# JettHuang/jet-pbrt

Hardware: AMD Instinct MI355X
Metric: Msamples/sec (whole node) + per-pixel L2 vs CPU ref, cornell_box 1024spp (higher is better)
Workload: dtype f32

## Files before the change

jet-pbrt_amd/csrc/jp_kernels.hip:

```cpp
#include "jp_common.h"
#include "jp_tex.h"
#include "jp_normals.h"
#include "jp_normal_map.h"
#include "jp_env.h"
#include "jp_mis.h"
#include "jp_lens.h"
#include "jp_xbsdf.h"
#include "jp_film.h"

#include <cstdio>
#include <cstring>
#include <string>
#include <vector>
#include <algorithm>
#include <cmath>
#include <mutex>
#include <thread>
#include "jp_devmem.h"
#include "jp_lbvh.h"
#include "jp_ploc.h"

struct NoLens {};
template <bool kLens> struct LensArg { typedef NoLens type; };
template <> struct LensArg<true> { typedef JpLensPlan type; };
// ... 155 lines not shown
		const float4 co = ro, cd = rd;
		if (j + JP_BLOCK < n) { ro = q.ray_o[cur][i + JP_BLOCK]; rd = q.ray_d[cur][i + JP_BLOCK]; }
		float tmax = JP_INF;
		int hit;
		if constexpr (kMode == 2) hit = acc.trace_unbounded(sc, xyz(co), xyz(cd), 0.001f, tmax);
		else hit = acc.template trace<false>(sc, xyz(co), xyz(cd), 0.001f, tmax);
		q.hit[i] = make_float2(tmax, __int_as_float(hit));
		h += hit >= 0 ? 1u : 0u;
	}
	for (int off = 32; off > 0; off >>= 1) h += __shfl_down(h, off);
	if ((threadIdx.x & 63) == 0 && h) atomicAdd(&cnt->closest_hit, (unsigned long long)h);
}

#ifndef JP_SHADE_TILE
#define JP_SHADE_TILE 8192
#endif
template <bool kSmooth> struct SmoothVars { };
template <> struct SmoothVars<true> { float4 next, rec; V3 Ns; bool on, guard; };
template <bool kSmooth> __device__ __forceinline__ V3 shade_n(const SmoothVars<kSmooth>& sm, V3 N) { if constexpr (kSmooth) return sm.Ns; else return N; }
template <bool kSmooth> __device__ __forceinline__ bool shade_refuses(const SmoothVars<kSmooth>& sm, V3 w, V3 wo, V3 Ng)
{
	if constexpr (kSmooth) return sm.guard && dot(w, Ng) * dot(wo, Ng) <= 0.f; else return false;
}
template <bool kTab, bool kPrims, bool kStage, bool kSort, bool kTex, bool kPick, bool kEnv, bool kMis, typename F = FeatAll, bool kOne = false, bool kSmooth = false>
__device__ __forceinline__ void shade_body(SceneView sc, Queues q, RenderConst rc, int cur, DevCounters* cnt, const TexView& tv, const PickView& pv, const EnvView& ev, const MisView& mv, const NormView& nv = NormView())
{
	static_assert(kPick || !kMis, "k_shade: the light strategy's pdf needs the light table");
	static_assert(kTab || !kPrims, "k_shade: primitive records in LDS only together with the tables");
	static_assert(kPick || !kEnv, "k_shade: the map light is an entry of the light table");
	static_assert(!kSmooth || !kPrims, "k_shade: a shading normal has no entry in the frame table");
	constexpr int kWaves = JP_BLOCK / 64, kMaxSeg = (JP_SHADE_TILE / JP_BLOCK) * kWaves;
	static_assert(JP_SHADE_TILE % JP_BLOCK == 0 && JP_SHADE_TILE <= 65536, "k_shade: tile positions are 16-bit");
	__shared__ unsigned short s_idx[kSort ? JP_SHADE_TILE : 1];
	static_assert(!kOne || (kSort && kPrims && !F::delta && !F::other_lights && !kTex && !kPick && !kMis), "k_shade: the one-sweep partition is the lean sorted instance's");
	__shared__ unsigned char s_key[kSort && !kOne ? JP_SHADE_TILE : 1];
	__shared__ unsigned int s_cnt[kSort && !kOne ? JP_SHADE_CLASSES * kMaxSeg : 1];
	__shared__ unsigned int s_two;
	__shared__ unsigned int s_wsum[kWaves];
	__shared__ unsigned int s_ctr[3];
	const unsigned int lane = threadIdx.x & 63u;
	const int n_tab_l = kPick ? 0 : 2 * sc.n_lights;
	const int n_tab = n_tab_l + 4 * sc.n_mats + (sc.n_mats + 3) / 4, n_tab_all = n_tab + (kPrims ? 8 * sc.n_prims : 0);
	float4* s_lights = s_dyn;
	float4* s_mats = s_lights + n_tab_l;
	int* s_mtype = (int*)(s_mats + 4 * sc.n_mats);
	float4* s_prims = s_dyn + n_tab;
	int4* s_meta = (int4*)(s_prims + 4 * sc.n_prims);
	const float4* s_frames = s_prims + 5 * sc.n_prims;
	float4* s_stage = s_dyn + n_tab_all + threadIdx.x;
	const unsigned int b = blockIdx.x, n = q.blk_q[cur][b];
	const int nxt = cur ^ 1;
#ifdef JP_SHADE_TIMING
	unsigned long long t_acc[10] = { 0, 0, 0, 0, 0, 0, 0, 0, 0, 0 }, t_last = __builtin_amdgcn_s_memtime();
#endif
	if (kTab)
	{
		for (int i = threadIdx.x; i < n_tab_all; i += 2 * JP_BLOCK)
		{
			const bool two = i + JP_BLOCK < n_tab_all;
			const float4 a = sc.shade_tab[i], c2 = two ? sc.shade_tab[i + JP_BLOCK] : a;
			s_dyn[i] = a; if (two) s_dyn[i + JP_BLOCK] = c2;
		}
	}
	if (n == 0) { if (threadIdx.x == 0) { q.blk_q[nxt][b] = 0; q.blk_sh[b] = 0; } return; }
	if (threadIdx.x == 0) { s_ctr[0] = 0; s_ctr[1] = 0; s_ctr[2] = 0; if (kOne) s_two = 0; }
	__syncthreads();
	const float4* lights = (kTab && !kPick) ? (const float4*)s_lights : sc.lights;
	const float4* mats = kTab ? (const float4*)s_mats : sc.mats;
	const int* mat_type = kTab ? (const int*)s_mtype : sc.mat_type;
	const float4* prims = kPrims ? (const float4*)s_prims : sc.prims;
	const int4* meta_t = kPrims ? (const int4*)s_meta : sc.meta;
	const unsigned int rbase = b * q.R;
	const unsigned int t0 = 0, count = n;
	JP_TS(0);
	if (kOne)
	{
		const unsigned int tid = threadIdx.x, npass = (count + JP_BLOCK - 1) / JP_BLOCK;
		const unsigned long long ltm = (1ull << lane) - 1ull;
		#pragma unroll 1
		for (unsigned int r0 = 0; r0 < npass; r0 += 8)
		{
			int pi[8];
			#pragma unroll
			for (int u = 0; u < 8; u++)
			{
				const unsigned int j = (r0 + u) * JP_BLOCK + tid;
				pi[u] = j < count ? __float_as_int(q.hit[rbase + t0 + j].y) : -2;
			}
			int mt[8]; unsigned long long ma[8], mb[8];
			unsigned int na = 0, nb = 0;
			#pragma unroll
			for (int u = 0; u < 8; u++)
			{
				mt[u] = -1;
				if (pi[u] >= 0) { const int m = meta_t[pi[u]].y; if (m >= 0) mt[u] = mat_type[m]; }
				ma[u] = __ballot(mt[u] == JP_MAT_MATTE); mb[u] = __ballot(mt[u] == JP_MAT_METAL);
				na += (unsigned int)__popcll(ma[u]); nb += (unsigned int)__popcll(mb[u]);
			}
// ... 74 lines not shown
			for (int i = 0; i < 3; i++) { const unsigned int at = 3 * tid + i; if (at < nctr) s_cnt[at] = base; base += v[i]; }
		}
		__syncthreads();
		#pragma unroll 1
		for (unsigned int r = 0; r < npass; r++)
		{
			const unsigned int key = s_key[r * JP_BLOCK + tid];
			unsigned int pre = 0;
			#pragma unroll
			for (int c = 0; c < JP_SHADE_CLASSES; c++)
			{
				if (!((rc.class_mask >> c) & 1)) continue;
				const unsigned long long m = __ballot(key == (unsigned int)c);
				if (key == (unsigned int)c) pre = (unsigned int)__popcll(m & ltm);
			}
			if (key < JP_SHADE_CLASSES) s_idx[s_cnt[key * seg + r * kWaves + wave] + pre] = (unsigned short)(r * JP_BLOCK + tid);
		}
		__syncthreads();
	}
	SmoothVars<kSmooth> sm;
	if constexpr (kSmooth) sm.next = make_float4(0, 0, 0, 0);
	float4 ro_n = make_float4(0, 0, 0, 0), rd_n = ro_n, rb_n = ro_n; float2 h_n = make_float2(0, 0); unsigned int s_n = 0; float2 m_n = make_float2(0, 0);
	JP_TS(1);
	const unsigned int n_front = kOne ? (s_two & 0xffffu) : 0u, n_back = kOne ? (s_two >> 16) : 0u, fence = ((n_front + 63u) >> 6) << 6;
#define JP_CHUNK_HAS(v)  (kOne ? ((v) < fence ? (v) < n_front : (v) - fence < n_back) : (v) < count)
#define JP_CHUNK_SPOT(v) (kOne ? ((v) < fence ? (v) : count - 1u - ((v) - fence)) : (v))
	const unsigned int nch = kOne ? (fence >> 6) + ((n_back + 63u) >> 6) : (count + 63u) >> 6;
	unsigned int tk = wave_take(&s_ctr[0], 1u);
	unsigned int c0 = (nch - 1u - tk) << 6;
	if (tk < nch && JP_CHUNK_HAS(c0 + lane)) { const unsigned int pos = JP_CHUNK_SPOT(c0 + lane), i0 = rbase + t0 + (kSort ? (unsigned int)s_idx[pos] : pos); ro_n = q.ray_o[cur][i0]; rd_n = q.ray_d[cur][i0]; rb_n = q.beta[cur][i0]; h_n = q.hit[i0]; if (kTex) s_n = tv.side[i0]; if (kMis) m_n = mv.side[cur][i0]; if constexpr (kSmooth) sm.next = nv.side[i0]; }
	while (tk < nch)
	{
		const bool valid = JP_CHUNK_HAS(c0 + lane);
#ifdef JP_SHADE_TIMING
		JP_TS(2);
		asm volatile("s_waitcnt vmcnt(0)" ::: "memory");
		JP_TS(3);
#endif
#ifdef JP_SHADE_NO_PREFETCH
		if (valid) { const unsigned int pos = JP_CHUNK_SPOT(c0 + lane), i0 = rbase + t0 + (kSort ? (unsigned int)s_idx[pos] : pos); ro_n = q.ray_o[cur][i0]; rd_n = q.ray_d[cur][i0]; rb_n = q.beta[cur][i0]; h_n = q.hit[i0]; if (kTex) s_n = tv.side[i0]; if (kMis) m_n = mv.side[cur][i0]; if constexpr (kSmooth) sm.next = nv.side[i0]; }
		const float4 ro = ro_n, rd = rd_n, rb = rb_n; const float2 h = h_n; const unsigned int sw = s_n; const float2 ms = m_n;
		if constexpr (kSmooth) sm.rec = sm.next;
		tk = wave_take(&s_ctr[0], 1u); c0 = (nch - 1u - tk) << 6;
#else
		const float4 ro = ro_n, rd = rd_n, rb = rb_n; const float2 h = h_n; const unsigned int sw = s_n; const float2 ms = m_n;
		if constexpr (kSmooth) sm.rec = sm.next;
		tk = wave_take(&s_ctr[0], 1u); c0 = (nch - 1u - tk) << 6;
		if (tk < nch && JP_CHUNK_HAS(c0 + lane))
		{
			const unsigned int pos = JP_CHUNK_SPOT(c0 + lane);
			const unsigned int i1 = rbase + t0 + (kSort ? (unsigned int)s_idx[pos] : pos);
			ro_n = q.ray_o[cur][i1]; rd_n = q.ray_d[cur][i1]; rb_n = q.beta[cur][i1]; h_n = q.hit[i1]; if (kTex) s_n = tv.side[i1]; if (kMis) m_n = mv.side[cur][i1]; if constexpr (kSmooth) sm.next = nv.side[i1];
		}
#endif
		bool shaded = false, wantNee = false, alive = false;
		V3 o = mk(0, 0, 0), d = mk(0, 0, 1), beta = mk(0, 0, 0), p = mk(0, 0, 0), N = mk(0, 0, 1);
		if constexpr (kSmooth) { sm.Ns = N; sm.on = false; sm.guard = false; }
		int slot = 0, bounce = 0; bool spec = false; unsigned int dim = 0; uint32_t key = 0;
		Closure c; c.kind = CL_LAMBERT; Frame fr; fr.s = fr.t = fr.n = mk(0, 0, 1);
		float2 nm = make_float2(0.f, 0.f);
		if (valid)
		{
			o = xyz(ro); d = xyz(rd); beta = xyz(rb);
			slot = __float_as_int(ro.w); key = (uint32_t)__float_as_int(rb.w);
			const int flags = __float_as_int(rd.w);
			bounce = FLAG_BOUNCE(flags); spec = FLAG_SPEC(flags); dim = FLAG_DIM(flags);
			const int pi = __float_as_int(h.y);
			const bool found = pi >= 0;
			int mat = -1, hitprim = 0; bool nflip = false, tabframe = kPrims;
			V3 Le = splat(0);
			float wLe = 1.f;
			if (found)
			{
				const float4 g3 = prims[4 * pi + 3];
				const int4 meta = meta_t[pi];
				const int type = __float_as_int(g3.w);
				p = o + h.x * d;
				if (type == JP_SHAPE_TRIANGLE) N = xyz(g3);
				else if (!F::curved || type == JP_SHAPE_RECTANGLE) { nflip = !(dot(xyz(g3), d) <= 0); N = nflip ? -xyz(g3) : xyz(g3); }
				else if (type == JP_SHAPE_DISK) N = xyz(prims[4 * pi + 1]);
				else { const float4 g0 = prims[4 * pi]; N = normalize(p - xyz(g0)); tabframe = false; }
				hitprim = pi;
// ... 55 lines not shown
					int l2; V3 Lr;
					if (kEnv) { l2 = ev.light; Lr = xyz(ev.texel[env_lookup(ev, d)]); }
					else { const float4 r4 = pv.env[e]; l2 = __float_as_int(r4.w); Lr = xyz(r4); }
					bool unweighed;
					const float a = light_pdf(sc, prims, lights, pv, ev, kEnv, l2, o, d, 0.f, N, unweighed);
					const float w = a > 0.f ? mis_weight(ms.x, a) : 1.f;
					float4 L = q.lacc[slot];
					V3 s2 = mk(L.x, L.y, L.z) + cmul(beta, Lr) * w;
					q.lacc[slot] = make_float4(s2.x, s2.y, s2.z, 0.f);
				}
			}
			if (!isblack(Le))
			{
				float4 L = q.lacc[slot];
				V3 a = mk(L.x, L.y, L.z) + (kMis ? cmul(beta, Le) * wLe : cmul(beta, Le));
				q.lacc[slot] = make_float4(a.x, a.y, a.z, 0.f);
			}
			if (found && bounce < rc.max_depth)
			{
				if (mat < 0) { alive = true; if (kMis) nm = make_float2(ms.x, ms.y + h.x); }
				else
				{
					float up = 0.f;
					const int mtype = mat_type[mat];
					if constexpr (kSmooth) { sm.on = sm.rec.w != 0.f; sm.Ns = sm.on ? xyz(sm.rec) : N; sm.guard = sm.on && mtype != JP_MAT_GLASS; }
					if (F::delta && mtype == JP_MAT_PLASTIC) up = rngf(rc, key, dim++);
					if (kTex && sw != 0u) make_closure_tex(mats, mtype, mat, up, tex_color(tv, sw), c);
					else make_closure<F>(mats, mtype, mat, up, c);
#ifdef JP_DBG_SKIP_FRAME
					fr.n = N; fr.s = mk(N.y, N.z, N.x); fr.t = mk(N.z, N.x, N.y);
#else
					if (kPrims && (!F::curved || tabframe))
					{
						const float4 fn = s_frames[3 * hitprim], fs = s_frames[3 * hitprim + 1], ft = s_frames[3 * hitprim + 2];
						fr.n = nflip ? -xyz(fn) : xyz(fn); fr.s = xyz(fs); fr.t = nflip ? -xyz(ft) : xyz(ft);
					}
					else fr = frame_from_z(shade_n<kSmooth>(sm, N));
#endif
					shaded = true;
					wantNee = !is_delta<F>(c);
#ifdef JP_DBG_SKIP_NEE
					wantNee = false;
#endif
				}
			}
		}
		JP_TS(4);
// ... 118 lines not shown
				for (int kk = 0; kk < k; kk++)
				{
					q.sh_d[(size_t)kk * q.cap + qs] = s_stage[(2 * kk) * JP_BLOCK];
					q.sh_c[(size_t)kk * q.cap + qs] = s_stage[(2 * kk + 1) * JP_BLOCK];
				}
			}
		}
		else if (ma) j = rbase + wave_take(&s_ctr[1], (unsigned int)__popcll(ma)) + (unsigned int)__popcll(ma & lt);
		if (alive)
		{
			q.ray_o[nxt][j] = make_float4(p.x, p.y, p.z, __int_as_float(slot));
			q.ray_d[nxt][j] = make_float4(nd.x, nd.y, nd.z, __int_as_float(MK_FLAGS(nbounce, nspec, dim)));
			q.beta[nxt][j] = make_float4(nbeta.x, nbeta.y, nbeta.z, __int_as_float((int)key));
			if (kMis) mv.side[nxt][j] = nm;
		}
		JP_TS(7);
#ifdef JP_SHADE_TIMING
		asm volatile("s_waitcnt vmcnt(0)" ::: "memory");
		JP_TS(9);
#endif
	}
#undef JP_CHUNK_HAS
#undef JP_CHUNK_SPOT
	JP_TS(2);
	__syncthreads();
	JP_TS(8);
#ifdef JP_SHADE_TIMING
	if (lane == 0) for (int i = 0; i < 10; i++) atomicAdd(&g_shade_t[i], t_acc[i]);
	if (lane == 0) atomicAdd(&g_shade_t[15], 1ull);
#endif
	if (threadIdx.x == 0)
	{
		const unsigned int run_q = kStage ? (s_ctr[1] & 0xffffu) : s_ctr[1], run_sh = kStage ? (s_ctr[1] >> 16) : s_ctr[2];
		q.blk_q[nxt][b] = run_q; q.blk_sh[b] = run_sh;
		if (run_q) atomicAdd(&cnt->n_queue[nxt], run_q);
		if (run_sh) atomicAdd(&cnt->n_shadow, run_sh);
	}
}
template <bool kTab, bool kPrims, bool kStage, bool kSort, typename F = FeatAll>
__global__ void __launch_bounds__(JP_BLOCK) k_shade(SceneView sc, Queues q, RenderConst rc, int cur, DevCounters* cnt)
{
	const TexView tv = {}; const PickView pv = {}; const EnvView ev = {}; const MisView mv = {};
	shade_body<kTab, kPrims, kStage, kSort, false, false, false, false, F>(sc, q, rc, cur, cnt, tv, pv, ev, mv);
}
__global__ void __launch_bounds__(JP_BLOCK) k_shade_lean_one(SceneView sc, Queues q, RenderConst rc, int cur, DevCounters* cnt)
{
	const TexView tv = {}; const PickView pv = {}; const EnvView ev = {}; const MisView mv = {};
	shade_body<true, true, true, true, false, false, false, false, FeatLean, true>(sc, q, rc, cur, cnt, tv, pv, ev, mv);
}

template <int kMode, typename F = FeatAll>
__global__ void __launch_bounds__(JP_BLOCK, 4) k_shadow(SceneView sc, Queues q, RenderConst rc, int depth, DevCounters* cnt)
{
#ifdef JP_TRAV_TIMING
	unsigned long long t_acc[10] = { 0, 0, 0, 0, 0, 0, 0, 0, 0, 0 }, t_last = __builtin_amdgcn_s_memtime();
#endif
	SceneAccess<kMode, F> acc(sc, depth);
	const unsigned int b = blockIdx.x, E = q.blk_sh[b], rbase = b * q.R;
	JP_TT(0);
	unsigned int rays = 0, occ = 0;
	float4 so_n = make_float4(0, 0, 0, 0), sd_n = make_float4(0, 0, 1, 0);
	if (threadIdx.x < E) { so_n = q.sh_o[rbase + threadIdx.x]; sd_n = q.sh_d[rbase + threadIdx.x]; }
	for (unsigned int j = threadIdx.x; j < E; j += JP_BLOCK)
	{
		const unsigned int e = rbase + j;
#ifdef JP_TRAV_TIMING
		JP_TT(1);
		asm volatile("s_waitcnt vmcnt(0)" ::: "memory");
		JP_TT(2);
#endif
		const float4 so = so_n; float4 sd = sd_n;
// ... 583 lines not shown
```

jet-pbrt_amd/csrc/jp_render.h:

```cpp
#pragma once
namespace
{
enum { CLS_EXTEND = 0, CLS_SHADE = 1, CLS_SHADOW = 2, CLS_OTHER = 3, CLS_PATH = 4, CLS_NORMAL = 5, CLS_NMAP = 6, CLS_TEXEL = 7 };

int lens_plan_of(const JpContext* c, JpLensPlan& lp)
{
	std::memset(&lp, 0, sizeof(lp));
	if (!c->lens_on) return JP_OK;
	if (jp_lens_make_plan(&c->plan.sv.cam, &c->lens, &lp) != 0) return fail(JP_ERR_INVALID_ARGUMENT, "jp_set_lens: the uploaded camera's right / up vectors have no finite positive length");
	return JP_OK;
}

void free_queues(JpContext* c) { c->qb = QueueBufs(); c->cap = 0; c->planes_alloc = 0; c->blk_alloc = 0; }

int ensure_queues(JpContext* c, unsigned int cap, int planes, unsigned int nblocks)
{
	if (c->cap >= cap && c->planes_alloc >= planes && c->blk_alloc >= nblocks) return JP_OK;
	cap = std::max(cap, c->cap); planes = std::max(planes, c->planes_alloc); nblocks = std::max(nblocks, c->blk_alloc);
	free_queues(c);
	auto alloc = [](DevBuf& b, auto*& p, size_t bytes) { return reserve(b, p, bytes) == hipSuccess; };
	Queues& q = c->q; QueueBufs& qb = c->qb; bool ok = true;
	for (int b = 0; b < 2 && ok; b++) ok = alloc(qb.ray_o[b], q.ray_o[b], (size_t)cap * 16) && alloc(qb.ray_d[b], q.ray_d[b], (size_t)cap * 16) && alloc(qb.beta[b], q.beta[b], (size_t)cap * 16)
	                                       && alloc(qb.blk_q[b], q.blk_q[b], (size_t)nblocks * 4);
	ok = ok && alloc(qb.hit, q.hit, (size_t)cap * 8) && alloc(qb.lacc, q.lacc, (size_t)cap * 16) && alloc(qb.sh_o, q.sh_o, (size_t)cap * 16)
// ... 98 lines not shown
}

typedef void (*ShadowKernel)(SceneView, Queues, RenderConst, int, DevCounters*);
typedef void (*ShadowRefillKernel)(SceneView, Queues, RenderConst, int, int*, DevCounters*);
struct ShadowLaunch { ShadowRefillKernel refill; ShadowKernel plain; size_t lds; int words; bool cert_fell_back; };
template <int M> ShadowRefillKernel shadow_refill(const ScenePlan& p)
{
	static const ShadowRefillKernel k[3][2] = { { k_shadow_persist<M, 8, false>, k_shadow_persist<M, 8, true> }, { k_shadow_persist<M, 16, false>, k_shadow_persist<M, 16, true> }, { k_shadow_persist<M, 32, false>, k_shadow_persist<M, 32, true> } };
	return k[refill_row(p)][p.vote];
}
ShadowLaunch shadow_kernel(const ScenePlan& p, unsigned int R, bool generic)
{
	const int words = std::min(shadow_depth(p), p.stack_lds_words);
	const size_t plds = (size_t)words * JP_BLOCK * sizeof(int) + (((size_t)R * p.n_planes + 31) / 32) * 4 * (p.cert ? 2 : 1);
	if (lean_traversal(p, generic)) return { nullptr, k_shadow<2, FeatFlat>, p.lds_bytes, p.stack_depth, p.cert };
	if (!refill_walks(p) || plds > 64 * 1024)
		return { nullptr, p.trav_mode == 3 ? k_shadow<3> : (p.trav_mode == 5 ? k_shadow<5> : (p.trav_mode == 2 ? k_shadow<2> : (p.trav_mode == 1 ? k_shadow<1> : k_shadow<0>))), p.trav_mode == 3 ? p.lds_bytes_shadow : p.lds_bytes, p.stack_depth, p.cert };
	const ShadowRefillKernel k = p.trav_mode == 5 ? (p.cert ? shadow_refill<6>(p) : shadow_refill<5>(p)) : (p.q4_shadow ? shadow_refill<4>(p) : (p.trav_mode == 3 ? shadow_refill<3>(p) : shadow_refill<0>(p)));
	return { k, nullptr, plds, words, false };
}

typedef void (*ShadeKernel)(SceneView, Queues, RenderConst, int, DevCounters*);
typedef void (*ShadeTexKernel)(SceneView, Queues, RenderConst, int, DevCounters*, TexView);
struct ShadeKernels { ShadeKernel plain; ShadeTexKernel tex; };
template <bool kTab, bool kPrims, bool kStage> ShadeKernels shade_row(bool sort)
{
	ShadeKernels k = { sort ? k_shade<kTab, kPrims, kStage, true> : k_shade<kTab, kPrims, kStage, false>, sort ? k_shade_tex<kTab, kPrims, kStage, true> : k_shade_tex<kTab, kPrims, kStage, false> };
	return k;
}
ShadeKernels shade_kernels(const ScenePlan& p, bool generic)
{
	if (lean_shading(p, generic))
	{
		ShadeKernels k = shade_row<true, true, true>(p.shade_sort);
		k.plain = p.shade_sort ? k_shade<true, true, true, true, FeatLean> : k_shade<true, true, true, false, FeatLean>;
#ifndef JP_NO_ONE_SWEEP
		if (p.shade_sort && !p.has_null_material) k.plain = k_shade_lean_one;
#endif
		return k;
	}
	if (p.shade_prims_in_lds) return p.stage_nee ? shade_row<true, true, true>(p.shade_sort) : shade_row<true, true, false>(p.shade_sort);
	if (p.tables_in_lds) return p.stage_nee ? shade_row<true, false, true>(p.shade_sort) : shade_row<true, false, false>(p.shade_sort);
	return shade_row<false, false, false>(p.shade_sort);
}

typedef void (*ShadePickKernel)(SceneView, Queues, RenderConst, int, DevCounters*, PickView);
typedef void (*ShadePickTexKernel)(SceneView, Queues, RenderConst, int, DevCounters*, TexView, PickView);
struct ShadePickKernels { ShadePickKernel plain; ShadePickTexKernel tex; };
ShadePickKernels shade_pick_kernels(const ScenePlan& p);
typedef void (*ShadeEnvKernel)(SceneView, Queues, RenderConst, int, DevCounters*, PickView, EnvView);
typedef void (*ShadeEnvTexKernel)(SceneView, Queues, RenderConst, int, DevCounters*, TexView, PickView, EnvView);
struct ShadeEnvKernels { ShadeEnvKernel plain; ShadeEnvTexKernel tex; };
ShadeEnvKernels shade_env_kernels(const ScenePlan& p);
typedef void (*ShadeMisKernel)(SceneView, Queues, RenderConst, int, DevCounters*, PickView, MisView);
typedef void (*ShadeMisTexKernel)(SceneView, Queues, RenderConst, int, DevCounters*, TexView, PickView, MisView);
typedef void (*ShadeMisEnvKernel)(SceneView, Queues, RenderConst, int, DevCounters*, PickView, EnvView, MisView);
typedef void (*ShadeMisEnvTexKernel)(SceneView, Queues, RenderConst, int, DevCounters*, TexView, PickView, EnvView, MisView);
struct ShadeMisKernels { ShadeMisKernel pick; ShadeMisTexKernel pick_tex; ShadeMisEnvKernel env; ShadeMisEnvTexKernel env_tex; };
ShadeMisKernels shade_mis_kernels(const ScenePlan& p);
struct SmoothKernels
// ... 98 lines not shown
		}
		c->q.cap = cap; c->q.R = R;
		const bool tex = p.textured && rp->integrator == JP_INTEGRATOR_PATH;
		if (tex) if (const int e = reserve_idle(c, c->side, (size_t)cap * sizeof(unsigned int)); e != JP_OK) return e;
		TexView tv = p.tv; tv.side = c->side.get<unsigned int>();
		const bool mis = c->estimator == JP_ESTIMATOR_MIS && rp->integrator == JP_INTEGRATOR_PATH;
		MisView mv = {};
		if (mis) if (const int e = ensure_mis_side(c, cap, mv); e != JP_OK) return e;
		NormView nv = p.nv;
		if (smooth) if (const int e = ensure_normal_side(c, cap, nv); e != JP_OK) return e;
		if (const int e = reserve_idle(c, c->spill, spill_need(p, p.persist ? deepest_walk(p) : 0, G) * sizeof(int)); e != JP_OK) return e;
		if (const int e = reserve_idle(c, c->pix_acc, (size_t)npix * 16); e != JP_OK) return e;
		int* const d_spill = c->spill.get<int>(); float4* const d_pix_acc = c->pix_acc.get<float4>();

		RenderConst rc; rc.width = rp->width; rc.height = rp->height; rc.spp = rp->spp; rc.max_depth = rp->max_depth; rc.seed = rp->seed;
		rc.band_rows = sh.band; rc.shard_index = sh.index; rc.shard_count = sh.count; rc.npix = (int)npix; rc.local_rows = sh.lane_rows; rc.n_planes = p.n_planes;
		rc.lane_index = lane_index; rc.lane_count = lane_count; rc.lane_rows = lane_group; rc.class_mask = p.class_mask; rc.sampler_debug = rp->sampler_mode == JP_SAMPLER_DEBUG ? 1 : 0;
		rc.slot_bits = slot_bits;
		rc.tiled = 0;
		rc.compact = (p.trav_mode != 2 && p.trav_mode != 1 && npix % JP_BLOCK == 0) ? 1 : 0;
		if (c->opt.compact_regions != 0) rc.compact = (c->opt.compact_regions > 0 && npix % JP_BLOCK == 0) ? 1 : 0;
		const int grid = (int)G;
		const bool generic = c->opt.reserved[0] == 1;
		const ExtendLaunch ek = extend_kernel(p, generic); const ShadowLaunch sk = shadow_kernel(p, R, generic); const ShadeKernels hk = shade_kernels(p, generic); const OtherKernel ok = other_kernel(p);
		const ShadePickKernels pk = p.pick ? shade_pick_kernels(p) : ShadePickKernels{ nullptr, nullptr };
		const ShadeEnvKernels vk = p.env ? shade_env_kernels(p) : ShadeEnvKernels{ nullptr, nullptr };
		const ShadeMisKernels mk2 = mis ? shade_mis_kernels(p) : ShadeMisKernels{ nullptr, nullptr, nullptr, nullptr };
		const SmoothKernels nk = smooth ? shade_smooth_kernels(p) : SmoothKernels{};
		JpLensPlan lp;
		if (const int e = lens_plan_of(c, lp); e != JP_OK) return e;
		for (int s0 = 0; s0 < rp->spp; s0 += sbatch)
		{
			rc.s0 = s0; rc.sbatch = std::min(sbatch, rp->spp - s0);
			{
				Stamper t(c, CLS_OTHER);
				if (c->lens_on) hipLaunchKernelGGL(k_raygen<true>, dim3(grid), dim3(JP_BLOCK), 0, c->stream, p.sv, c->q, rc, d_cnt, lp);
				else hipLaunchKernelGGL(k_raygen<false>, dim3(grid), dim3(JP_BLOCK), 0, c->stream, p.sv, c->q, rc, d_cnt, NoLens());
			}
			if (rp->integrator != JP_INTEGRATOR_PATH)
			{
				Stamper t(c, CLS_OTHER);
				const int ogrid = (int)std::min<unsigned int>((P + JP_BLOCK - 1) / JP_BLOCK, (unsigned int)(c->n_cus * 16));
				hipLaunchKernelGGL(ok, dim3(ogrid), dim3(JP_BLOCK), p.lds_bytes, c->stream, p.sv, c->q, rc, rp->integrator, p.stack_depth, d_cnt, c->lens_on ? 1 : 0, lp);
			}
			int cur = 0;
			int iters = rp->integrator != JP_INTEGRATOR_PATH ? 0 : rp->max_depth + 1;
			for (int it = 0;; it++)
			{
				if (it >= iters)
				{
					if (rp->integrator != JP_INTEGRATOR_PATH || !p.has_null_material || it > iters + 64) break;
// ... 21 lines not shown
							else if (p.env) hipLaunchKernelGGL(nk.env_tex, dim3(grid), dim3(JP_BLOCK), l, c->stream, p.sv, c->q, rc, cur, d_cnt, tv, p.pv, p.ev, nv);
							else if (p.pick) hipLaunchKernelGGL(nk.pick_tex, dim3(grid), dim3(JP_BLOCK), l, c->stream, p.sv, c->q, rc, cur, d_cnt, tv, p.pv, nv);
							else hipLaunchKernelGGL(nk.tex, dim3(grid), dim3(JP_BLOCK), l, c->stream, p.sv, c->q, rc, cur, d_cnt, tv, nv);
						}
						else if (mis && p.env) hipLaunchKernelGGL(nk.mis_env, dim3(grid), dim3(JP_BLOCK), l, c->stream, p.sv, c->q, rc, cur, d_cnt, p.pv, p.ev, mv, nv);
						else if (mis) hipLaunchKernelGGL(nk.mis, dim3(grid), dim3(JP_BLOCK), l, c->stream, p.sv, c->q, rc, cur, d_cnt, p.pv, mv, nv);
						else if (p.env) hipLaunchKernelGGL(nk.env, dim3(grid), dim3(JP_BLOCK), l, c->stream, p.sv, c->q, rc, cur, d_cnt, p.pv, p.ev, nv);
						else if (p.pick) hipLaunchKernelGGL(nk.pick, dim3(grid), dim3(JP_BLOCK), l, c->stream, p.sv, c->q, rc, cur, d_cnt, p.pv, nv);
						else hipLaunchKernelGGL(nk.plain, dim3(grid), dim3(JP_BLOCK), l, c->stream, p.sv, c->q, rc, cur, d_cnt, nv);
					}
					else if (tex)
					{
						launch_texel(c, p, grid, cur, tv);
						if (mis && p.env) hipLaunchKernelGGL(mk2.env_tex, dim3(grid), dim3(JP_BLOCK), p.shade_lds_bytes, c->stream, p.sv, c->q, rc, cur, d_cnt, tv, p.pv, p.ev, mv);
						else if (mis) hipLaunchKernelGGL(mk2.pick_tex, dim3(grid), dim3(JP_BLOCK), p.shade_lds_bytes, c->stream, p.sv, c->q, rc, cur, d_cnt, tv, p.pv, mv);
						else if (p.env) hipLaunchKernelGGL(vk.tex, dim3(grid), dim3(JP_BLOCK), p.shade_lds_bytes, c->stream, p.sv, c->q, rc, cur, d_cnt, tv, p.pv, p.ev);
						else if (p.pick) hipLaunchKernelGGL(pk.tex, dim3(grid), dim3(JP_BLOCK), p.shade_lds_bytes, c->stream, p.sv, c->q, rc, cur, d_cnt, tv, p.pv);
						else hipLaunchKernelGGL(hk.tex, dim3(grid), dim3(JP_BLOCK), p.shade_lds_bytes, c->stream, p.sv, c->q, rc, cur, d_cnt, tv);
					}
					else if (mis && p.env) hipLaunchKernelGGL(mk2.env, dim3(grid), dim3(JP_BLOCK), p.shade_lds_bytes, c->stream, p.sv, c->q, rc, cur, d_cnt, p.pv, p.ev, mv);
					else if (mis) hipLaunchKernelGGL(mk2.pick, dim3(grid), dim3(JP_BLOCK), p.shade_lds_bytes, c->stream, p.sv, c->q, rc, cur, d_cnt, p.pv, mv);
					else if (p.env) hipLaunchKernelGGL(vk.plain, dim3(grid), dim3(JP_BLOCK), p.shade_lds_bytes, c->stream, p.sv, c->q, rc, cur, d_cnt, p.pv, p.ev);
					else if (p.pick) hipLaunchKernelGGL(pk.plain, dim3(grid), dim3(JP_BLOCK), p.shade_lds_bytes, c->stream, p.sv, c->q, rc, cur, d_cnt, p.pv);
					else hipLaunchKernelGGL(hk.plain, dim3(grid), dim3(JP_BLOCK), p.shade_lds_bytes, c->stream, p.sv, c->q, rc, cur, d_cnt);
				}
				HIP_TRY(hipGetLastError());
				if (it < rp->max_depth || p.has_null_material)
				{
					Stamper t(c, CLS_SHADOW);
					if (sk.cert_fell_back) c->cert_fell_back = true;
					if (sk.refill) hipLaunchKernelGGL(sk.refill, dim3(grid), dim3(JP_BLOCK), sk.lds, c->stream, p.sv, c->q, rc, sk.words, d_spill, d_cnt);
					else hipLaunchKernelGGL(sk.plain, dim3(grid), dim3(JP_BLOCK), sk.lds, c->stream, p.sv, c->q, rc, sk.words, d_cnt);
					HIP_TRY(hipGetLastError());
				}
				cur ^= 1;
			}
			{ Stamper t(c, CLS_OTHER); launch_resolve(c, c->q, rc, npix, d_pix_acc, film_dev, s0 == 0 ? 1 : 0, s0 + rc.sbatch >= rp->spp ? 1 : 0); }
			samples += (unsigned long long)rc.sbatch * (unsigned long long)npix;
		}
		HIP_TRY(hipGetLastError());
	}
	HIP_TRY(hipEventRecord(c->ev1, c->stream));
	c->own_samples = samples;
	if (sync) HIP_TRY(hipStreamSynchronize(c->stream));
	return JP_OK;
}
// ... 476 lines not shown
```

jet-pbrt_amd/csrc/jp_runtime.h:

```cpp
#pragma once

static thread_local std::string g_err;
static int fail(int code, const std::string& msg) { g_err = msg; return code; }
#define HIP_TRY(expr) do { hipError_t _e = (expr); if (_e != hipSuccess) return fail(JP_ERR_DEVICE, std::string(#expr) + ": " + hipGetErrorString(_e)); } while (0)

static inline bool opt_flag(int v, bool dflt) { return v == 0 ? dflt : v > 0; }

static void options_from_environment(JpOptions& o)
{
	struct Item { const char* name; int kind; void* field; int as; };
	const Item items[] = {
		{ "JETPBRT_LANES", 0, &o.lanes, 0 }, { "JETPBRT_LANE_ROWS", 0, &o.lane_rows, 0 }, { "JETPBRT_BLOCKS_PER_CU", 0, &o.blocks_per_cu, 0 }, { "JETPBRT_MAX_SLOTS", 3, &o.max_slots, 0 },
		{ "JETPBRT_COMPACT_REGIONS", 1, &o.compact_regions, 0 }, { "JETPBRT_FUSED", 1, &o.fused, 0 }, { "JETPBRT_REGION", 0, &o.fused_region, 0 }, { "JETPBRT_JOB_SPP", 0, &o.fused_job_spp, 0 },
		{ "JETPBRT_FUSED_WGS", 0, &o.fused_workgroups, 0 }, { "JETPBRT_TRAVERSAL", 6, &o.traversal, 0 }, { "JETPBRT_Q4", 1, &o.q4, 0 }, { "JETPBRT_Q4_SHADOW", 1, &o.q4_shadow, 0 },
		{ "JETPBRT_PERSIST", 2, &o.persist, 0 }, { "JETPBRT_VOTE", 1, &o.vote, 0 }, { "JETPBRT_STACK_LDS", 0, &o.stack_lds_words, 0 }, { "JETPBRT_SHADE_SORT", 1, &o.shade_sort, 0 },
		{ "JETPBRT_DEVICE_TREE", 4, &o.device_tree, 0 }, { "JETPBRT_DEVICE_WIDE", 1, &o.device_wide, 0 }, { "JETPBRT_BVH_MAXLEAF", 0, &o.bvh_max_leaf, 0 },
		{ "JETPBRT_PLOC_RADIUS", 0, &o.ploc_radius, 0 }, { "JETPBRT_PLOC_MAX_ROUNDS", 0, &o.ploc_max_rounds, 0 }, { "JETPBRT_CERTIFIED", 1, &o.certified, 0 },
		{ "JETPBRT_CERT_SLACK", 7, &o.cert_slack, 0 }, { "JETPBRT_CERT_SLACK_EYE", 7, &o.cert_slack_eye, 0 }, { "JETPBRT_CERT_EYE", 7, &o.cert_eye_tau, 0 },
		{ "JETPBRT_SINCOSF", 2, &o.libm_sincosf, 0 }, { "JETPBRT_LIBM", 2, &o.libm_xbsdf, 0 },
		{ "JETPBRT_TRACE_BINARY", 5, &o.trace_walk, 1 }, { "JETPBRT_TRACE_WIDE", 5, &o.trace_walk, 2 }, { "JETPBRT_TRACE_VERBATIM", 5, &o.trace_walk, 3 }, { "JETPBRT_BOX_PAD", 7, &o.box_pad, 0 },
	};
	for (const Item& it : items)
	{
		const char* e = getenv(it.name);
// ... 46 lines not shown
struct QueueBufs { DevBuf ray_o[2], ray_d[2], beta[2], blk_q[2], hit, lacc, sh_o, sh_d, sh_c, blk_sh; };

struct EnvMapHost { int W = 0, H = 0, up = 0, importance = 0; std::vector<float> rgb; };
struct VertexNormalsHost { bool set = false; int n_triangles = 0, n_smooth = 0; std::vector<float> vn; };

struct NormalMapsHost { bool set = false; int n_materials = 0, n_triangles = 0, n_mapped = 0; std::vector<int> width, height, mat_map; std::vector<long long> first; std::vector<char> neutral;
                        std::vector<unsigned int> texels; std::vector<float> strength, tri_uv; };

struct TexSamplingHost { bool has_tex = false, has_map = false; int n_textures = 0, n_maps = 0, n_active_textures = 0, n_active_maps = 0; std::vector<JpTexSampler> tex, map; };

struct JpContext
{
	int device = 0;
	JpOptions opt{}, opt_env{};
	hipStream_t stream = nullptr;
	int n_cus = 256;
	ScenePlan plan; SceneTables tab;
	bool cert_fell_back = false; int cert_eye_leaves = 0;
	int sincosf_mode = 0, libm_mode = 0;
	bool build_on_device = false; float build_ms = 0.f; int bvh_height = 0, bvh_nodes = 0;
	int wide_height = 0, q4_height = 0; size_t tab_bytes[JP_UPLOAD_TABLES] = {};
	Queues q = {}; QueueBufs qb; unsigned int cap = 0; int planes_alloc = 0; unsigned int blk_alloc = 0; int blocks_per_cu = 16;
	DevBuf pix_acc, spill, film;
	DevBuf bsdf_in, bsdf_out, bsdf_fl;
	DevBuf gamma, rgb8; PinnedBuf h_rgb8;
	PinnedBuf h_film;
	DevBuf cnt;
	hipEvent_t ev0 = nullptr, ev1 = nullptr;
	bool profiling = false;
	std::vector<hipEvent_t> evpool; size_t evused = 0;
	struct Stamp { int cls; size_t a, b; };
	std::vector<Stamp> stamps;
	JpCounters counters;
	std::vector<JpContext*> lanes; bool is_lane = false; unsigned long long own_samples = 0; bool bpc_from_env = false;
	hipEvent_t ev_added = nullptr; bool added_valid = false; int last_lanes = 1;
	Queues fq = {}; QueueBufs fqb; unsigned int fcap = 0; int fplanes = 0;
	DevBuf jobs;
	int last_fused = 0, last_region = 0, last_wgs = 0;
	int n_textures = 0, n_tex_mats = 0; long long texel_bytes = 0; int last_textured = 0;
	DevBuf side;
	DevBuf dn_cz[2], dn_nr, dn_stage;
	hipEvent_t dn_ev[2] = { nullptr, nullptr }, gd_ev[2] = { nullptr, nullptr }; bool dn_timed = false, gd_timed = false;
	int last_dn = 0, last_dn_demod = 0, last_guide_spp = 0; float last_dn_sigma[3] = { 0.f, 0.f, 0.f };
	int light_mode = JP_LIGHTS_ALL;
	int n_selectable = 0; double total_weight = 0.0; int last_picked = 0;
	EnvMapHost env_map;
// ... 255 lines not shown
```

Measured before the change: 3328.

## Split lean one-sweep shade kernel into matte and metal specialised launches

Measured after the change: 3336 (median of 2 runs). Within noise of the previous version (+0.2%).

```diff
diff --git a/jet-pbrt_amd/csrc/jp_kernels.hip b/jet-pbrt_amd/csrc/jp_kernels.hip
--- a/jet-pbrt_amd/csrc/jp_kernels.hip
+++ b/jet-pbrt_amd/csrc/jp_kernels.hip
@@ -201,16 +201,18 @@
 {
 	if constexpr (kSmooth) return sm.guard && dot(w, Ng) * dot(wo, Ng) <= 0.f; else return false;
 }
-template <bool kTab, bool kPrims, bool kStage, bool kSort, bool kTex, bool kPick, bool kEnv, bool kMis, typename F = FeatAll, bool kOne = false, bool kSmooth = false>
-__device__ __forceinline__ void shade_body(SceneView sc, Queues q, RenderConst rc, int cur, DevCounters* cnt, const TexView& tv, const PickView& pv, const EnvView& ev, const MisView& mv, const NormView& nv = NormView())
-{
+struct SplitView { unsigned short* list; unsigned int* count; };
+template <bool kTab, bool kPrims, bool kStage, bool kSort, bool kTex, bool kPick, bool kEnv, bool kMis, typename F = FeatAll, bool kOne = false, bool kSmooth = false, int kSplit = 0>
+__device__ __forceinline__ void shade_body(SceneView sc, Queues q, RenderConst rc, int cur, DevCounters* cnt, const TexView& tv, const PickView& pv, const EnvView& ev, const MisView& mv, const NormView& nv = NormView(), const SplitView& sl = SplitView())
+{
+	static_assert(kSplit == 0 || (kOne && kStage && !kSmooth), "k_shade: the matte / metal pair is the one-sweep instance split in two");
 	static_assert(kPick || !kMis, "k_shade: the light strategy's pdf needs the light table");
 	static_assert(kTab || !kPrims, "k_shade: primitive records in LDS only together with the tables");
 	static_assert(kPick || !kEnv, "k_shade: the map light is an entry of the light table");
 	static_assert(!kSmooth || !kPrims, "k_shade: a shading normal has no entry in the frame table");
 	constexpr int kWaves = JP_BLOCK / 64, kMaxSeg = (JP_SHADE_TILE / JP_BLOCK) * kWaves;
 	static_assert(JP_SHADE_TILE % JP_BLOCK == 0 && JP_SHADE_TILE <= 65536, "k_shade: tile positions are 16-bit");
-	__shared__ unsigned short s_idx[kSort ? JP_SHADE_TILE : 1];
+	__shared__ unsigned short s_idx[kSort && kSplit != 2 ? JP_SHADE_TILE : 1];
 	static_assert(!kOne || (kSort && kPrims && !F::delta && !F::other_lights && !kTex && !kPick && !kMis), "k_shade: the one-sweep partition is the lean sorted instance's");
 	__shared__ unsigned char s_key[kSort && !kOne ? JP_SHADE_TILE : 1];
 	__shared__ unsigned int s_cnt[kSort && !kOne ? JP_SHADE_CLASSES * kMaxSeg : 1];
@@ -227,8 +229,9 @@
 	int4* s_meta = (int4*)(s_prims + 4 * sc.n_prims);
 	const float4* s_frames = s_prims + 5 * sc.n_prims;
 	float4* s_stage = s_dyn + n_tab_all + threadIdx.x;
-	const unsigned int b = blockIdx.x, n = q.blk_q[cur][b];
+	const unsigned int b = blockIdx.x, n = kSplit == 2 ? sl.count[b] : q.blk_q[cur][b];
 	const int nxt = cur ^ 1;
+	if (kSplit == 2 && n == 0) return;
 #ifdef JP_SHADE_TIMING
 	unsigned long long t_acc[10] = { 0, 0, 0, 0, 0, 0, 0, 0, 0, 0 }, t_last = __builtin_amdgcn_s_memtime();
 #endif
@@ -241,8 +244,13 @@
 			s_dyn[i] = a; if (two) s_dyn[i + JP_BLOCK] = c2;
 		}
 	}
-	if (n == 0) { if (threadIdx.x == 0) { q.blk_q[nxt][b] = 0; q.blk_sh[b] = 0; } return; }
-	if (threadIdx.x == 0) { s_ctr[0] = 0; s_ctr[1] = 0; s_ctr[2] = 0; if (kOne) s_two = 0; }
+	if (kSplit != 2 && n == 0) { if (threadIdx.x == 0) { q.blk_q[nxt][b] = 0; q.blk_sh[b] = 0; if (kSplit == 1) sl.count[b] = 0; } return; }
+	unsigned int fill0 = 0;
+	if (threadIdx.x == 0)
+	{
+		if (kSplit == 2) fill0 = q.blk_q[nxt][b] | (q.blk_sh[b] << 16);
+		s_ctr[0] = 0; s_ctr[1] = fill0; s_ctr[2] = 0; if (kOne) s_two = 0;
+	}
 	__syncthreads();
 	const float4* lights = (kTab && !kPick) ? (const float4*)s_lights : sc.lights;
 	const float4* mats = kTab ? (const float4*)s_mats : sc.mats;
@@ -252,7 +260,8 @@
 	const unsigned int rbase = b * q.R;
 	const unsigned int t0 = 0, count = n;
 	JP_TS(0);
-	if (kOne)
+	if (kOne && kSplit == 2) { }
+	else if (kOne)
 	{
 		const unsigned int tid = threadIdx.x, npass = (count + JP_BLOCK - 1) / JP_BLOCK;
 		const unsigned long long ltm = (1ull << lane) - 1ull;
@@ -373,13 +382,20 @@
 	if constexpr (kSmooth) sm.next = make_float4(0, 0, 0, 0);
 	float4 ro_n = make_float4(0, 0, 0, 0), rd_n = ro_n, rb_n = ro_n; float2 h_n = make_float2(0, 0); unsigned int s_n = 0; float2 m_n = make_float2(0, 0);
 	JP_TS(1);
-	const unsigned int n_front = kOne ? (s_two & 0xffffu) : 0u, n_back = kOne ? (s_two >> 16) : 0u, fence = ((n_front + 63u) >> 6) << 6;
+	const unsigned int n_front = kSplit == 2 ? n : (kOne ? (s_two & 0xffffu) : 0u), n_back = (kOne && kSplit == 0) ? (s_two >> 16) : 0u, fence = ((n_front + 63u) >> 6) << 6;
+	if (kSplit == 1)
+	{
+		const unsigned int n_metal = s_two >> 16;
+		for (unsigned int i = threadIdx.x; i < n_metal; i += JP_BLOCK) sl.list[rbase + i] = s_idx[count - 1u - i];
+		if (threadIdx.x == 0) sl.count[b] = n_metal;
+	}
 #define JP_CHUNK_HAS(v)  (kOne ? ((v) < fence ? (v) < n_front : (v) - fence < n_back) : (v) < count)
-#define JP_CHUNK_SPOT(v) (kOne ? ((v) < fence ? (v) : count - 1u - ((v) - fence)) : (v))
+#define JP_CHUNK_SPOT(v) (kOne ? ((kSplit != 0 || (v) < fence) ? (v) : count - 1u - ((v) - fence)) : (v))
+#define JP_CHUNK_AT(pos) (kSplit == 2 ? (unsigned int)sl.list[rbase + (pos)] : (kSort ? (unsigned int)s_idx[pos] : (pos)))
 	const unsigned int nch = kOne ? (fence >> 6) + ((n_back + 63u) >> 6) : (count + 63u) >> 6;
 	unsigned int tk = wave_take(&s_ctr[0], 1u);
 	unsigned int c0 = (nch - 1u - tk) << 6;
-	if (tk < nch && JP_CHUNK_HAS(c0 + lane)) { const unsigned int pos = JP_CHUNK_SPOT(c0 + lane), i0 = rbase + t0 + (kSort ? (unsigned int)s_idx[pos] : pos); ro_n = q.ray_o[cur][i0]; rd_n = q.ray_d[cur][i0]; rb_n = q.beta[cur][i0]; h_n = q.hit[i0]; if (kTex) s_n = tv.side[i0]; if (kMis) m_n = mv.side[cur][i0]; if constexpr (kSmooth) sm.next = nv.side[i0]; }
+	if (tk < nch && JP_CHUNK_HAS(c0 + lane)) { const unsigned int pos = JP_CHUNK_SPOT(c0 + lane), i0 = rbase + t0 + JP_CHUNK_AT(pos); ro_n = q.ray_o[cur][i0]; rd_n = q.ray_d[cur][i0]; rb_n = q.beta[cur][i0]; h_n = q.hit[i0]; if (kTex) s_n = tv.side[i0]; if (kMis) m_n = mv.side[cur][i0]; if constexpr (kSmooth) sm.next = nv.side[i0]; }
 	while (tk < nch)
 	{
 		const bool valid = JP_CHUNK_HAS(c0 + lane);
@@ -389,7 +405,7 @@
 		JP_TS(3);
 #endif
 #ifdef JP_SHADE_NO_PREFETCH
-		if (valid) { const unsigned int pos = JP_CHUNK_SPOT(c0 + lane), i0 = rbase + t0 + (kSort ? (unsigned int)s_idx[pos] : pos); ro_n = q.ray_o[cur][i0]; rd_n = q.ray_d[cur][i0]; rb_n = q.beta[cur][i0]; h_n = q.hit[i0]; if (kTex) s_n = tv.side[i0]; if (kMis) m_n = mv.side[cur][i0]; if constexpr (kSmooth) sm.next = nv.side[i0]; }
+		if (valid) { const unsigned int pos = JP_CHUNK_SPOT(c0 + lane), i0 = rbase + t0 + JP_CHUNK_AT(pos); ro_n = q.ray_o[cur][i0]; rd_n = q.ray_d[cur][i0]; rb_n = q.beta[cur][i0]; h_n = q.hit[i0]; if (kTex) s_n = tv.side[i0]; if (kMis) m_n = mv.side[cur][i0]; if constexpr (kSmooth) sm.next = nv.side[i0]; }
 		const float4 ro = ro_n, rd = rd_n, rb = rb_n; const float2 h = h_n; const unsigned int sw = s_n; const float2 ms = m_n;
 		if constexpr (kSmooth) sm.rec = sm.next;
 		tk = wave_take(&s_ctr[0], 1u); c0 = (nch - 1u - tk) << 6;
@@ -400,7 +416,7 @@
 		if (tk < nch && JP_CHUNK_HAS(c0 + lane))
 		{
 			const unsigned int pos = JP_CHUNK_SPOT(c0 + lane);
-			const unsigned int i1 = rbase + t0 + (kSort ? (unsigned int)s_idx[pos] : pos);
+			const unsigned int i1 = rbase + t0 + JP_CHUNK_AT(pos);
 			ro_n = q.ray_o[cur][i1]; rd_n = q.ray_d[cur][i1]; rb_n = q.beta[cur][i1]; h_n = q.hit[i1]; if (kTex) s_n = tv.side[i1]; if (kMis) m_n = mv.side[cur][i1]; if constexpr (kSmooth) sm.next = nv.side[i1];
 		}
 #endif
@@ -408,7 +424,7 @@
 		V3 o = mk(0, 0, 0), d = mk(0, 0, 1), beta = mk(0, 0, 0), p = mk(0, 0, 0), N = mk(0, 0, 1);
 		if constexpr (kSmooth) { sm.Ns = N; sm.on = false; sm.guard = false; }
 		int slot = 0, bounce = 0; bool spec = false; unsigned int dim = 0; uint32_t key = 0;
-		Closure c; c.kind = CL_LAMBERT; Frame fr; fr.s = fr.t = fr.n = mk(0, 0, 1);
+		Closure c; c.kind = kSplit == 2 ? CL_MICROFACET : CL_LAMBERT; Frame fr; fr.s = fr.t = fr.n = mk(0, 0, 1);
 		float2 nm = make_float2(0.f, 0.f);
 		if (valid)
 		{
@@ -510,7 +526,7 @@
 				else
 				{
 					float up = 0.f;
-					const int mtype = mat_type[mat];
+					const int mtype = kSplit == 1 ? JP_MAT_MATTE : (kSplit == 2 ? JP_MAT_METAL : mat_type[mat]);
 					if constexpr (kSmooth) { sm.on = sm.rec.w != 0.f; sm.Ns = sm.on ? xyz(sm.rec) : N; sm.guard = sm.on && mtype != JP_MAT_GLASS; }
 					if (F::delta && mtype == JP_MAT_PLASTIC) up = rngf(rc, key, dim++);
 					if (kTex && sw != 0u) make_closure_tex(mats, mtype, mat, up, tex_color(tv, sw), c);
@@ -675,6 +691,7 @@
 	}
 #undef JP_CHUNK_HAS
 #undef JP_CHUNK_SPOT
+#undef JP_CHUNK_AT
 	JP_TS(2);
 	__syncthreads();
 	JP_TS(8);
@@ -686,8 +703,9 @@
 	{
 		const unsigned int run_q = kStage ? (s_ctr[1] & 0xffffu) : s_ctr[1], run_sh = kStage ? (s_ctr[1] >> 16) : s_ctr[2];
 		q.blk_q[nxt][b] = run_q; q.blk_sh[b] = run_sh;
-		if (run_q) atomicAdd(&cnt->n_queue[nxt], run_q);
-		if (run_sh) atomicAdd(&cnt->n_shadow, run_sh);
+		const unsigned int add_q = run_q - (fill0 & 0xffffu), add_sh = run_sh - (fill0 >> 16);
+		if (add_q) atomicAdd(&cnt->n_queue[nxt], add_q);
+		if (add_sh) atomicAdd(&cnt->n_shadow, add_sh);
 	}
 }
 template <bool kTab, bool kPrims, bool kStage, bool kSort, typename F = FeatAll>
@@ -700,6 +718,16 @@
 {
 	const TexView tv = {}; const PickView pv = {}; const EnvView ev = {}; const MisView mv = {};
 	shade_body<true, true, true, true, false, false, false, false, FeatLean, true>(sc, q, rc, cur, cnt, tv, pv, ev, mv);
+}
+__global__ void __launch_bounds__(JP_BLOCK, 4) k_shade_lean_matte(SceneView sc, Queues q, RenderConst rc, int cur, DevCounters* cnt, SplitView sl)
+{
+	const TexView tv = {}; const PickView pv = {}; const EnvView ev = {}; const MisView mv = {};
+	shade_body<true, true, true, true, false, false, false, false, FeatLean, true, false, 1>(sc, q, rc, cur, cnt, tv, pv, ev, mv, NormView(), sl);
+}
+__global__ void __launch_bounds__(JP_BLOCK, 3) k_shade_lean_metal(SceneView sc, Queues q, RenderConst rc, int cur, DevCounters* cnt, SplitView sl)
+{
+	const TexView tv = {}; const PickView pv = {}; const EnvView ev = {}; const MisView mv = {};
+	shade_body<true, true, true, true, false, false, false, false, FeatLean, true, false, 2>(sc, q, rc, cur, cnt, tv, pv, ev, mv, NormView(), sl);
 }
 
 template <int kMode, typename F = FeatAll>
diff --git a/jet-pbrt_amd/csrc/jp_render.h b/jet-pbrt_amd/csrc/jp_render.h
--- a/jet-pbrt_amd/csrc/jp_render.h
+++ b/jet-pbrt_amd/csrc/jp_render.h
@@ -144,13 +144,14 @@
 
 typedef void (*ShadeKernel)(SceneView, Queues, RenderConst, int, DevCounters*);
 typedef void (*ShadeTexKernel)(SceneView, Queues, RenderConst, int, DevCounters*, TexView);
-struct ShadeKernels { ShadeKernel plain; ShadeTexKernel tex; };
+typedef void (*ShadeSplitKernel)(SceneView, Queues, RenderConst, int, DevCounters*, SplitView);
+struct ShadeKernels { ShadeKernel plain; ShadeTexKernel tex; ShadeSplitKernel matte = nullptr, metal = nullptr; };
 template <bool kTab, bool kPrims, bool kStage> ShadeKernels shade_row(bool sort)
 {
 	ShadeKernels k = { sort ? k_shade<kTab, kPrims, kStage, true> : k_shade<kTab, kPrims, kStage, false>, sort ? k_shade_tex<kTab, kPrims, kStage, true> : k_shade_tex<kTab, kPrims, kStage, false> };
 	return k;
 }
-ShadeKernels shade_kernels(const ScenePlan& p, bool generic)
+ShadeKernels shade_kernels(const ScenePlan& p, bool generic, bool pair = false)
 {
 	if (lean_shading(p, generic))
 	{
@@ -158,6 +159,14 @@
 		k.plain = p.shade_sort ? k_shade<true, true, true, true, FeatLean> : k_shade<true, true, true, false, FeatLean>;
 #ifndef JP_NO_ONE_SWEEP
 		if (p.shade_sort && !p.has_null_material) k.plain = k_shade_lean_one;
+#ifndef JP_NO_SPLIT_SHADE
+		const bool matte = (p.class_mask & (2 << JP_MAT_MATTE)) != 0, metal = (p.class_mask & (2 << JP_MAT_METAL)) != 0;
+#ifdef JP_SPLIT_SHADE_PAIR
+		pair = true;
+#endif
+		if (!p.has_null_material && matte && !metal) k.matte = k_shade_lean_matte;
+		else if (!p.has_null_material && matte && metal && p.shade_sort && pair) { k.matte = k_shade_lean_matte; k.metal = k_shade_lean_metal; }
+#endif
 #endif
 		return k;
 	}
@@ -302,11 +311,17 @@
 		if (c->opt.compact_regions != 0) rc.compact = (c->opt.compact_regions > 0 && npix % JP_BLOCK == 0) ? 1 : 0;
 		const int grid = (int)G;
 		const bool generic = c->opt.reserved[0] == 1;
-		const ExtendLaunch ek = extend_kernel(p, generic); const ShadowLaunch sk = shadow_kernel(p, R, generic); const ShadeKernels hk = shade_kernels(p, generic); const OtherKernel ok = other_kernel(p);
+		const ExtendLaunch ek = extend_kernel(p, generic); const ShadowLaunch sk = shadow_kernel(p, R, generic); const ShadeKernels hk = shade_kernels(p, generic, c->opt.reserved[0] == 2); const OtherKernel ok = other_kernel(p);
 		const ShadePickKernels pk = p.pick ? shade_pick_kernels(p) : ShadePickKernels{ nullptr, nullptr };
 		const ShadeEnvKernels vk = p.env ? shade_env_kernels(p) : ShadeEnvKernels{ nullptr, nullptr };
 		const ShadeMisKernels mk2 = mis ? shade_mis_kernels(p) : ShadeMisKernels{ nullptr, nullptr, nullptr, nullptr };
 		const SmoothKernels nk = smooth ? shade_smooth_kernels(p) : SmoothKernels{};
+		SplitView sl = { nullptr, nullptr };
+		if (hk.matte)
+		{
+			if (const int e = reserve_idle(c, c->split, (size_t)cap * sizeof(unsigned short) + (size_t)G * sizeof(unsigned int)); e != JP_OK) return e;
+			sl.list = c->split.get<unsigned short>(); sl.count = (unsigned int*)(sl.list + cap);
+		}
 		JpLensPlan lp;
 		if (const int e = lens_plan_of(c, lp); e != JP_OK) return e;
 		for (int s0 = 0; s0 < rp->spp; s0 += sbatch)
@@ -374,6 +389,11 @@
 					else if (mis) hipLaunchKernelGGL(mk2.pick, dim3(grid), dim3(JP_BLOCK), p.shade_lds_bytes, c->stream, p.sv, c->q, rc, cur, d_cnt, p.pv, mv);
 					else if (p.env) hipLaunchKernelGGL(vk.plain, dim3(grid), dim3(JP_BLOCK), p.shade_lds_bytes, c->stream, p.sv, c->q, rc, cur, d_cnt, p.pv, p.ev);
 					else if (p.pick) hipLaunchKernelGGL(pk.plain, dim3(grid), dim3(JP_BLOCK), p.shade_lds_bytes, c->stream, p.sv, c->q, rc, cur, d_cnt, p.pv);
+					else if (hk.matte)
+					{
+						hipLaunchKernelGGL(hk.matte, dim3(grid), dim3(JP_BLOCK), p.shade_lds_bytes, c->stream, p.sv, c->q, rc, cur, d_cnt, sl);
+						if (hk.metal) hipLaunchKernelGGL(hk.metal, dim3(grid), dim3(JP_BLOCK), p.shade_lds_bytes, c->stream, p.sv, c->q, rc, cur, d_cnt, sl);
+					}
 					else hipLaunchKernelGGL(hk.plain, dim3(grid), dim3(JP_BLOCK), p.shade_lds_bytes, c->stream, p.sv, c->q, rc, cur, d_cnt);
 				}
 				HIP_TRY(hipGetLastError());
diff --git a/jet-pbrt_amd/csrc/jp_runtime.h b/jet-pbrt_amd/csrc/jp_runtime.h
--- a/jet-pbrt_amd/csrc/jp_runtime.h
+++ b/jet-pbrt_amd/csrc/jp_runtime.h
@@ -92,6 +92,7 @@
 	int wide_height = 0, q4_height = 0; size_t tab_bytes[JP_UPLOAD_TABLES] = {};
 	Queues q = {}; QueueBufs qb; unsigned int cap = 0; int planes_alloc = 0; unsigned int blk_alloc = 0; int blocks_per_cu = 16;
 	DevBuf pix_acc, spill, film;
+	DevBuf split;
 	DevBuf bsdf_in, bsdf_out, bsdf_fl;
 	DevBuf gamma, rgb8; PinnedBuf h_rgb8;
 	PinnedBuf h_film;
```
